# troyvvgroup/quemb

Hardware: AMD Instinct MI355X
Metric: fragment CCSD iters/sec (full BE sweep over synthetic n_occ=20 n_virt=200 fragments); corr-E error vs oracle in parity_max_abs_err_Eh / parity_n220_abs_err_Eh (higher is better)
Workload: dtype f64

## Files before the change

### include/qemb_hip_ops.h

```cpp
#ifndef QEMB_HIP_OPS_H
#define QEMB_HIP_OPS_H
#include "qemb_hip.h"
#ifdef __cplusplus
extern "C" {
#endif

#define QEMB_TIMER_LADDER 0
#define QEMB_TIMER_RINGS 1
#define QEMB_TIMER_ITER 2
#define QEMB_TIMER_AO2MO 3
#define QEMB_TIMER_SCF 4
#define QEMB_TIMER_GEMM_ANY 5
#define QEMB_TIMER_SCHMIDT 6
#define QEMB_TIMER_DF 7
int qemb_timer_begin(int slot);
int qemb_timer_end(int slot);
int qemb_timer_read(int slot, double* total_ms, int64_t* count);
int qemb_timer_reset(int slot);
int qemb_alloc_stats(long long* n_driver_allocs, long long* n_driver_frees, double* ms_in_driver_calls, double* gb_allocated, int reset);
int qemb_gemm_flop_count(double* flops, int reset);
int qemb_tape_cache_counters(int64_t* reused, int64_t* recorded, int reset);
int qemb_ctx_timer_read(int ctx, int slot, double* total_ms, int64_t* count, int reset);
int qemb_timer_live_events(int slot);

// ... 35 lines not shown
int qemb_op_unpack_s4(int64_t n, const double* s4, double* s1);
int qemb_op_pack_s4(int64_t n, const double* s1, double* s4);
int qemb_op_unpack_s8_to_s4(int64_t n, const double* s8, double* s4);
int qemb_op_mirror_lower(int64_t n, double* A, int64_t lda);
int qemb_op_k_from_pairs(int64_t n, const double* H, const double* D, double* K);
int qemb_op_jk_from_packed(int64_t n, const double* S4, const double* D, const double* Dp, double* Jp, double* K);
int qemb_op_pack_pm_cols(int64_t rows, int64_t v, const double* in, double* Op, int64_t ldp, double* Om, int64_t ldm);
int qemb_op_scatter_pm_rows(int64_t o, int64_t ncols, const double* Xp, const double* Xm, double* out);
int qemb_op_pack_w_pm(int64_t o, const double* W, double* Ap, int64_t lda_p, double* Am, int64_t lda_m);
int qemb_op_ladder_scatter_pm2(int64_t o, int64_t v, const double* Rp, int64_t ldp, const double* Rm, int64_t ldm, const double* Hp, const double* Hm,
                               int assign, double* t2);
int qemb_op_lincomb2(int64_t n, double a, const double* x, double b, const double* y, double beta, double* out);
int qemb_op_small_k_update(int64_t batch, int64_t M, int64_t N, int64_t K, double alpha, const double* A, int64_t sA, const double* B, int64_t sB, double* C, int64_t sC);
int qemb_op_ccsd_ph_layouts(int64_t o, int64_t v, const double* t2, const double* t1, double* T, double* Tp, double* S, double* Ut, double* Tpt, double* Th);
int qemb_op_ccsd_y_traces(int64_t o, int64_t v, const double* ZC, const double* ZB, double* Y);
int qemb_op_copy4_two(const int64_t dim[4], const double* in, const int64_t si[4], double* out, const int64_t so[4], double alpha, double beta, const double* base,
                      double* out2, const double* in2, double c2a, double c2b);
int qemb_op_scatter_pm_rows_add(int64_t o, int64_t ncols, const double* Xp, const double* Xm, double* out, const double* add);
int qemb_op_ccsd_y_traces_add(int64_t o, int64_t v, const double* ZC, const double* ZB, double* Y, const double* add);
int qemb_op_pack_w_pm_sum(int64_t o, const double* Wt, const double* X, const double* At, double* Ap, int64_t lda_p, double* Am, int64_t lda_m);
int qemb_op_ccsd_t1_small(int64_t o, int64_t v, const double* t1, const double* Lvv, const double* Loo, const double* Fov, double* t1n);
int qemb_op_ccsd_t1_assemble(int64_t o, int64_t v, const double* t1, const double* Lvv, const double* Loo, const double* Fov, const double* S, const double* Lph1,
                             const double* PA, int SA, int64_t strideA, const double* PB, int SB, int64_t strideB, double* t1n);
int qemb_op_gemv_rows_two(int64_t rows1, int64_t cols1, const double* T1, int64_t ld1, const double* x1, double* y1, double a1, double b1,
                          int64_t rows2, int64_t cols2, const double* T2, int64_t ld2, const double* x2, double* y2, double a2, double b2);
int qemb_op_ccsd_y_traces_slabs(int64_t o, int64_t v, const double* ZC, const double* ZB, double* Y, const double* add, int S, int64_t stride, double scale);
int qemb_op_gemv_rows2(int64_t rows, int64_t cols, const double* T1, int64_t ld1, const double* x1, const double* T2, int64_t ld2, const double* x2, double* y, double alpha, double beta);
int qemb_op_ccsd_finish_t2_rings(int64_t o, int64_t v, double* t2n, const double* U, const double* OV, const double* RS, const double* M, const double* eo, const double* ev, double* t1n);
int qemb_op_diis_push(int64_t n, const double* trial, const double* prev, double* e, double* xcopy, int m, const double* const* ys, int self, double* row_dev, double* row_host);
int qemb_op_ccsd_extrapolate_energy(int64_t o, int64_t v, int nterms, const double* coef, const double* const* xs, double* amp, const double* L, double* tau, double* e_host);
// ... 82 lines not shown
```

### quemb_amd/_lib.py

```python

from __future__ import annotations

import ctypes as C
import os
from pathlib import Path

import numpy as np

_HERE = Path(__file__).resolve().parent
LIB_PATH = _HERE / "libqemb_hip.so"

c_dp = C.POINTER(C.c_double)
c_i64 = C.c_int64
c_vp = C.c_void_p


QEMB_ERR_ARG, QEMB_ERR_ALLOC, QEMB_ERR_DEVICE, QEMB_ERR_NOCONV, QEMB_ERR_NUMERIC, QEMB_ERR_UNSUPPORTED = -1, -2, -3, -4, -5, -6


class QembError(RuntimeError):

    def __init__(self, msg="", status=None):
        super().__init__(msg)
        self.status = status
# ... 77 lines not shown
    f("qemb_op_unpack_s4", I, L, P, P)
    f("qemb_op_pack_s4", I, L, P, P)
    f("qemb_op_unpack_s8_to_s4", I, L, P, P)
    f("qemb_op_unpack_tril_rows", I, L, L, P, P)
    f("qemb_op_pack_pair_rows", I, L, L, P, P)
    f("qemb_op_mirror_lower", I, L, P, L)
    f("qemb_op_k_from_pairs", I, L, P, P, P)
    f("qemb_op_jk_from_packed", I, L, P, P, P, P, P)
    f("qemb_op_pack_pm_cols", I, L, L, P, P, L, P, L)
    f("qemb_op_scatter_pm_rows", I, L, L, P, P, P)
    f("qemb_op_pack_w_pm", I, L, P, P, L, P, L)
    f("qemb_op_ladder_scatter_pm2", I, L, L, P, L, P, L, P, P, I, P)
    f("qemb_op_lincomb2", I, L, D, P, D, P, D, P)
    f("qemb_op_small_k_update", I, L, L, L, L, D, P, L, P, L, P, L)
    f("qemb_op_ccsd_ph_layouts", I, L, L, P, P, P, P, P, P, P, P)
    f("qemb_op_ccsd_y_traces", I, L, L, P, P, P)
    f("qemb_op_copy4_two", I, C.POINTER(L), P, C.POINTER(L), P, C.POINTER(L), D, D, P, P, P, D, D)
    f("qemb_op_scatter_pm_rows_add", I, L, L, P, P, P, P)
    f("qemb_op_ccsd_y_traces_add", I, L, L, P, P, P, P)
    f("qemb_op_pack_w_pm_sum", I, L, P, P, P, P, L, P, L)
    f("qemb_op_ccsd_t1_small", I, L, L, P, P, P, P, P)
    f("qemb_op_gemv_rows2", I, L, L, P, L, P, P, L, P, P, D, D)
    f("qemb_op_ccsd_t1_assemble", I, L, L, P, P, P, P, P, P, P, I, L, P, I, L, P)
    f("qemb_op_gemv_rows_two", I, L, L, P, L, P, P, D, D, L, L, P, L, P, P, D, D)
    f("qemb_op_ccsd_y_traces_slabs", I, L, L, P, P, P, P, I, L, D)
    f("qemb_op_ccsd_finish_t2_rings", I, L, L, P, P, P, P, P, P, P, P)
    f("qemb_op_diis_push", I, L, P, P, P, P, I, P, I, P, P)
    f("qemb_op_ccsd_extrapolate_energy", I, L, L, I, P, P, P, P, P, P)
    f("qemb_op_gather_rows", I, L, L, P, P, L, P)
    f("qemb_op_scale_rows", I, L, L, P, P)
# ... 250 lines not shown
```

### quemb_amd/csrc/api.cpp

```cpp
#include <cstring>
#include <cstdlib>
#include <vector>
#include <execinfo.h>
#include <signal.h>
#include <unistd.h>
#include "../../include/qemb_hip_ops.h"
#include "dev_ops.h"
#include "ccsd.h"
#include "fragment.h"
#include "ao2mo.h"
#include "kdf.h"
#include "int3c.h"
#include "int4c.h"
#include "cd_core.h"
#include "loc_core.h"
#include "sci_core.h"
#include <algorithm>
#include <cmath>
#include <mutex>
#include <set>

using namespace qemb;
namespace qemb {
int dev_mfma_f64_peak(int iters, int blocks_per_cu, double* tflops);
// ... 183 lines not shown
int qemb_op_pack_w_pm(int64_t o, const double* W, double* Ap, int64_t lda_p, double* Am, int64_t lda_m) { return dev_pack_w_pm(o, W, Ap, lda_p, Am, lda_m); }
int qemb_op_ladder_scatter_pm2(int64_t o, int64_t v, const double* Rp, int64_t ldp, const double* Rm, int64_t ldm, const double* Hp, const double* Hm,
                               int assign, double* t2) { return dev_ladder_scatter_pm2(o, v, Rp, ldp, Rm, ldm, Hp, Hm, assign, t2); }
int qemb_op_lincomb2(int64_t n, double a, const double* x, double b, const double* y, double beta, double* out) {
  const double c[2] = {a, b};
  const double* xs[2] = {x, y};
  return dev_lincomb(n, 2, c, xs, beta, out);
}
int qemb_op_mirror_lower(int64_t n, double* A, int64_t lda) { return dev_mirror_lower(n, A, lda); }
int qemb_op_small_k_update(int64_t batch, int64_t M, int64_t N, int64_t K, double alpha, const double* A, int64_t sA, const double* B, int64_t sB, double* C, int64_t sC) {
  return dev_small_k_update(batch, M, N, K, alpha, A, sA, B, sB, C, sC);
}
int qemb_op_ccsd_ph_layouts(int64_t o, int64_t v, const double* t2, const double* t1, double* T, double* Tp, double* S, double* Ut, double* Tpt, double* Th) {
  return dev_ccsd_ph_layouts(o, v, t2, t1, T, Tp, S, Ut, Tpt, Th);
}
int qemb_op_copy4_two(const int64_t dim[4], const double* in, const int64_t si[4], double* out, const int64_t so[4], double alpha, double beta, const double* base,
                      double* out2, const double* in2, double c2a, double c2b) {
  Copy4Desc c{};
  for (int k = 0; k < 4; ++k) { c.dim[k] = dim[k]; c.si[k] = si[k]; c.so[k] = so[k]; }
  c.in = in; c.out = out; c.alpha = alpha; c.beta = beta; c.base = base;
  c.out2 = out2; c.in2 = in2; c.c2a = c2a; c.c2b = c2b;
  return dev_copy4(c);
}
int qemb_op_scatter_pm_rows_add(int64_t o, int64_t ncols, const double* Xp, const double* Xm, double* out, const double* add) { return dev_scatter_pm_rows(o, ncols, Xp, Xm, out, add); }
int qemb_op_ccsd_y_traces_add(int64_t o, int64_t v, const double* ZC, const double* ZB, double* Y, const double* add) { return dev_ccsd_y_traces(o, v, ZC, ZB, Y, add); }
int qemb_op_pack_w_pm_sum(int64_t o, const double* Wt, const double* X, const double* At, double* Ap, int64_t lda_p, double* Am, int64_t lda_m) {
  return dev_pack_w_pm_sum(o, Wt, X, At, Ap, lda_p, Am, lda_m);
}
int qemb_op_ccsd_t1_small(int64_t o, int64_t v, const double* t1, const double* Lvv, const double* Loo, const double* Fov, double* t1n) { return dev_ccsd_t1_small(o, v, t1, Lvv, Loo, Fov, t1n); }
int qemb_op_ccsd_t1_assemble(int64_t o, int64_t v, const double* t1, const double* Lvv, const double* Loo, const double* Fov, const double* S, const double* Lph1,
// ... 1064 lines not shown
```

### quemb_amd/csrc/ccsd.cpp

```cpp
#include "ccsd.h"
#include "ao2mo.h"
#include <algorithm>
#include <chrono>
#include <cmath>
#include <cstdio>
#include <cstdlib>
#include <cstring>
#include <string>

namespace qemb {

int mo_slab_ld(int n) { return (n >= 64 && n <= 1024) ? (n + 15) / 16 * 16 : n; }
int64_t mo_transform_work(int n) { return (int64_t)n * mo_slab_ld(n) * ((int64_t)n * (n + 1) / 2); }

static int mo_three_quarter_blocks(int n, int o, int nf, const double* T, int64_t slab, MoIntegrals& out, bool build_T34) {
  const int v = n - o;
  if (nf > 0 && build_T34) {
    QTRY(out.T34.alloc((int64_t)n * n * n * nf));
    QTRY(dev_extract_pf_t(n, T, 0, 0, 0, 0, n, n, n, nf, out.T34, slab));
  } else if (nf > 0) {
    QTRY(out.A1.alloc((int64_t)v * o * v * nf));
    QTRY(out.A2.alloc((int64_t)o * o * v * nf));
    QTRY(dev_extract_pf_t(n, T, o, 0, o, 0, v, o, v, nf, out.A1, slab));
    QTRY(dev_extract_pf_t(n, T, 0, 0, o, 0, o, o, v, nf, out.A2, slab));
// ... 133 lines not shown
    QTRY(mo_blocks_from_pair_product(n, o, X1, X0, out));
    QTRY(lap_AO2MO.close());
    return 0;
  }
  QTRY(dev_unpack_tril_rows(np, n, X1, X0));
  if (nf > 0) {
    QTRY(gemm(np, (int64_t)nf * n, naux, 1.0, Lpk, np, false, Lh, n2, false, 0.0, X1, (int64_t)nf * n));
    QTRY(mo_three_quarter_blocks(n, o, nf, X1, (int64_t)nf * n, out, build_T34));
  }
  Lh.release(); Lpk.release();
  QTRY(mo_blocks_from_pair_first(n, o, X0, X1, mo_transform_work(n), out, build_Vl));
  QTRY(lap_AO2MO.close());
  return 0;
}

int CcsdSolver::setup(MoIntegrals&& ints, const double* mo_energy_dev) {
  I_ = std::move(ints);
  o_ = I_.o; v_ = I_.v; nf_ = I_.nf;
  const int64_t o = o_, v = v_, nov = o * v, oo = o * o, vv = v * v, N2 = oo * vv;
  QTRY(eo_.alloc(o)); QTRY(ev_.alloc(v));
  QTRY(dev_d2d(eo_, mo_energy_dev, sizeof(double) * o));
  QTRY(dev_d2d(ev_, mo_energy_dev + o, sizeof(double) * v));
  QTRY(ovov_t_.alloc(nov * nov)); QTRY(Lovov_.alloc(nov * nov)); QTRY(Loovv_.alloc(N2)); QTRY(OVoovv_.alloc(N2));
  QTRY(Lovoo_.alloc(o * v * oo)); QTRY(W1base_.alloc(N2)); QTRY(W2base_.alloc(N2)); QTRY(Lph1_.alloc(N2));
  QTRY(oooo_p_.alloc(oo * oo));
  QTRY(perm4(ovov_t_, I_.ovov, o, v, o, v, 0, 3, 2, 1));
  QTRY(dcopy(nov * nov, I_.ovov, Lovov_));
  QTRY(axpby(nov * nov, -1.0, ovov_t_, 2.0, Lovov_));
  QTRY(perm4(Loovv_, Lovov_, o, v, o, v, 0, 2, 1, 3));
  QTRY(perm4(OVoovv_, I_.ovov, o, v, o, v, 0, 2, 1, 3));
// ... 25 lines not shown
    if (I_.ovvv_pk.p) ovvv_pk_ = std::move(I_.ovvv_pk);
    else { QTRY(ovvv_pk_.alloc(o * v * npv)); QTRY(dev_pack_tril_rows(o * v, v, I_.ovvv, ovvv_pk_)); }
  }
  QTRY(Gp_.alloc(oo * I_.ldp)); QTRY(Gm_.alloc(oo * I_.ldm));
  QTRY(dev_pack_pm_cols(oo, v, OVoovv_, Gp_, I_.ldp, Gm_, I_.ldm));
  QTRY(perm4(oooo_p_, I_.oooo, o, o, o, o, 1, 3, 0, 2));
  QTRY(ovoo_cikl_.alloc(v * oo * o));
  QTRY(perm4(ovoo_cikl_, I_.ovoo, o, v, o, o, 1, 3, 2, 0));
  const int64_t na = nov + N2;
  QTRY(amp_.alloc(na)); QTRY(ampn_.alloc(na)); QTRY(diff_.alloc(na));
  for (DBuf* b : {&tau_, &T_, &Tp_, &S_, &W1_, &W2_, &W12_, &W12b_, &R_, &U_}) QTRY(b->alloc(N2));
  const int64_t NG = std::max<int64_t>(N2, oo * o * v);
  QTRY(G2_.alloc(NG));
  plans_ = ccsd_gemm_plans(o, v);
  QTRY(Fvv_.alloc(plans_.fvv.elems()));
  QTRY(T1P_.alloc(plans_.pa.elems() + plans_.pb.elems()));
  QTRY(Foo_.alloc(oo)); QTRY(Fov_.alloc(nov)); QTRY(Z_.alloc(oo)); QTRY(Y_.alloc(vv));
  QTRY(Ytmp_.alloc(vv)); QTRY(Loo_.alloc(oo)); QTRY(Lvv_.alloc(vv)); QTRY(Q_.alloc(oo)); QTRY(Wo_.alloc(oo * oo));
  QTRY(O1_.alloc(oo * oo)); QTRY(X_.alloc(oo * nov)); QTRY(scal_.alloc(8));
  {
    const int64_t npo = o * (o + 1) / 2, nmo = std::max<int64_t>(o * (o - 1) / 2, 1);
    QTRY(LTp_.alloc(npo * I_.ldp)); QTRY(LRp_.alloc(std::max(npo * I_.ldp, plans_.ladder_p.elems())));
    QTRY(LTm_.alloc(nmo * I_.ldm)); QTRY(LRm_.alloc(std::max(nmo * I_.ldm, plans_.ladder_m.elems())));
    QTRY(Xp_.alloc(plans_.x_p.elems())); QTRY(Xm_.alloc(plans_.x_m.elems()));
    QTRY(Xwp_.alloc(plans_.xw_p.elems())); QTRY(Xwm_.alloc(plans_.xw_m.elems())); QTRY(Xw_.alloc(oo * oo));
    lwp_ = npo + (npo & 1); lwm_ = std::max<int64_t>(2, nmo + (nmo & 1));
    QTRY(WAp_.alloc(npo * lwp_)); QTRY(WAm_.alloc(nmo * lwm_)); QTRY(HRp_.alloc(npo * I_.ldp)); QTRY(HRm_.alloc(nmo * I_.ldm));
    QTRY(ZB_.alloc(N2)); QTRY(ZC_.alloc(N2));
  }
  first_ = true;
  return 0;
// ... 70 lines not shown
}
static GemmPlan pick_xw_split(int64_t rows, int64_t oo, int64_t K) {
  if (K < 2048) return GemmPlan(rows, oo, K, -1, 0);
  const int cfg = GEMM_64x64;
  const int64_t tiles = gemm_tile_count(cfg, rows, oo);
  return GemmPlan(rows, oo, K, cfg, (int)std::max<int64_t>(1, std::min<int64_t>(std::min<int64_t>(64, K / 256), (512 + tiles - 1) / tiles)));
}
static GemmPlan pick_long_k(int64_t M, int64_t N, int64_t K, int cfg, bool many_slices = false) {
  if (cfg < 0) return GemmPlan(M, N, K, cfg, 0);
  int ks = gemm_auto_ksplit(gemm_tile_count(cfg, M, N), K);
  if (many_slices && ks > 1 && M <= 32 && N <= 32) ks = (int)std::min<int64_t>(512, K / 64);
  return GemmPlan(M, N, K, cfg, ks);
}
static int tile_tall(int64_t o) { return (o <= 32) ? GEMM_128x32 : -1; }
static int tile_wide(int64_t o) { return (o <= 32) ? GEMM_32x128 : -1; }

CcsdGemmPlans ccsd_gemm_plans(int64_t o, int64_t v) {
  int64_t ldp, ldm;
  packed_pair_lds(v, ldp, ldm);
  const int64_t oo = o * o, vv = v * v, nov = o * v;
  const int64_t npo = o * (o + 1) / 2, nmo = std::max<int64_t>(o * (o - 1) / 2, 1), npv = v * (v + 1) / 2, nmv = std::max<int64_t>(v * (v - 1) / 2, 1);
  CcsdGemmPlans p;
  p.fvv = pick_long_k(v, v, oo * v, (v <= 256) ? GEMM_64x64 : -1);
  p.pa = pick_long_k(o, v, o * vv, tile_wide(o), true);
  p.pb = pick_long_k(o, v, o * v * o, tile_wide(o), true);
  p.ladder_p = pick_pair_gemm(npo, npv, ldp);
  p.ladder_m = pick_pair_gemm(nmo, nmv, ldm);
  p.xw_p = pick_xw_split(npo, oo, ldp);
  p.xw_m = pick_xw_split(nmo, oo, ldm);
  p.x_p = pick_pair_gemm(npo, nov, ldp, true);
// ... 25 lines not shown
      if (nmo > 0 && nmv > 0) QTRY(gemm(nmo, nmv, nmo, 1.0, WAm_, lwm_, true, LTm_, ldm, false, 0.0, HRm_, ldm, 1, 0, 0, 0, nmv >= 2048 ? tile_for(nmo) : -1));
      QTRY(dev_region_end());
      QTRY(dev_ladder_scatter_pm2(o, v, LRp_, sp.ld, LRm_, sm.ld, HRp_, (nmo > 0 && nmv > 0) ? HRm_.p : nullptr, 1, out, sp.S, sp.stride, sm.S, sm.stride, ldp, ldm));
    } else {
      QTRY(dev_ladder_scatter_pm2(o, v, LRp_, sp.ld, LRm_, sm.ld, nullptr, nullptr, 0, out, sp.S, sp.stride, sm.S, sm.stride));
    }
  }
  return 0;
}

int CcsdSolver::update_amps(double* t1n, double* t2n) {
  const int64_t o = o_, v = v_, nov = o * v, oo = o * o, vv = v * v;
  const double* t1 = this->t1();
  const double* t2 = this->t2();
  QTRY(dev_region_begin());
  QTRY(dev_ccsd_ph_layouts(o, v, t2, t1, T_, Tp_, S_, W12_, W12b_, R_));
  QTRY(dev_region_chain());
  QTRY(dev_ladder_pack_tau(o, v, tau_, LTp_, I_.ldp, LTm_, I_.ldm));
  QTRY(dev_region_end());

  {
    const int64_t nmo = o * (o - 1) / 2, nmv = v * (v - 1) / 2;
    SlabGemm sp, sm;
    QTRY(dev_region_begin());
    QTRY(gemm_slabs(plans_.xw_p, LTp_, I_.ldp, Gp_, I_.ldp, Xwp_, oo, sp));
    QTRY(dev_region_chain());
    if (nmo > 0) {
      if (nmv > 0) QTRY(gemm_slabs(plans_.xw_m, LTm_, I_.ldm, Gm_, I_.ldm, Xwm_, oo, sm));
      else QTRY(dev_fill(Xwm_, nmo * oo, 0.0));
    }
    QTRY(dev_region_end());
    QTRY(dev_scatter_pm_rows(o, oo, Xwp_, Xwm_, Xw_, nullptr, sp.S, sp.stride, sm.S, sm.stride));
  }
  QTRY(dev_foo_from_x(o, Xw_, Loo_));
  SlabGemm sfvv;
  double fvv_scale = -1.0;
  if (plans_.fvv.ks > 1) QTRY(gemm_slabs(plans_.fvv, tau_, v, Loovv_, v, Fvv_, v, sfvv, false, false));
  else { QTRY(gemm(v, v, oo * v, -1.0, tau_, v, false, Loovv_, v, false, 0.0, Fvv_, v, 1, 0, 0, 0, plans_.fvv.cfg)); fvv_scale = 1.0; }
  QTRY(dev_gemv_rows_two(nov, nov, Lovov_, nov, t1, Fov_, 1.0, 0.0, oo, nov, LovooT_, nov, t1, Loo_, 1.0, 1.0));
  const int cfg_tall = tile_tall(o), cfg_wide = tile_wide(o);
  QTRY(dev_region_begin());
  QTRY(gemm(o * vv, o, v, 1.0, I_.ovvv, v, true, t1, v, true, 0.0, ZB_, o, 1, 0, 0, 0, cfg_tall));
  QTRY(dev_region_chain());
  {
    const int64_t npv = v * (v + 1) / 2;
    const bool vec_ok = (npv % 2) == 0;
    QTRY(gemm(o, npv, v, 1.0, t1, v, true, ovvv_pk_, npv, false, 0.0, ZCp_, npv, o, 0, v * npv, o * npv, vec_ok ? cfg_wide : -1));
    QTRY(dev_unpack_tril_rows(oo, v, ZCp_, ZC_));
  }
  QTRY(dev_region_end());
  QTRY(dev_ccsd_y_traces(o, v, ZC_, ZB_, Lvv_, Fvv_, sfvv.S, sfvv.stride, fvv_scale));

  SlabGemm spa, spb;
  double* PA = T1P_.p;
  QTRY(dev_region_begin());
  QTRY(gemm_slabs(plans_.pa, R_, o * vv, I_.ovvv, v, PA, v, spa, true, false));
  double* PB = PA + (int64_t)spa.S * nov;
  QTRY(dev_region_chain());
  QTRY(gemm_slabs(plans_.pb, Lovoo_, o, T_, v, PB, v, spb, false, false));
  QTRY(dev_region_end());
  QTRY(dev_ccsd_t1_assemble(o, v, t1, Lvv_, Loo_, Fov_, S_, Lph1_, PA, spa.S, nov, PB, spb.S, nov, t1n));

  QTRY(gemm(o, oo * o, v, 1.0, t1, v, true, ovoo_cikl_, oo * o, false, 0.0, O1_, oo * o));
  QTRY(dev_pack_w_pm_sum(o, oooo_p_, Xw_, O1_, WAp_, lwp_, WAm_, lwm_));
  QTRY(apply_ladder(tau_, t2n, true, true));

  QTRY(gemm(oo * v, v, v, 1.0, t2, v, true, Lvv_, v, true, 0.0, U_, v));
  QTRY(gemm(o, o * vv, o, -1.0, Loo_, o, false, t2, o * vv, false, 1.0, U_, o * vv, 1, 0, 0, 0, cfg_wide));
  {
    const int64_t nmo = o * (o - 1) / 2;
    SlabGemm sp, sm;
    QTRY(dev_region_begin());
    QTRY(gemm_slabs(plans_.x_p, LTp_, I_.ldp, OVp_, I_.ldp, Xp_, nov, sp));
    QTRY(dev_region_chain());
    if (nmo > 0) QTRY(gemm_slabs(plans_.x_m, LTm_, I_.ldm, OVm_, I_.ldm, Xm_, nov, sm));
// ... 324 lines not shown
```

### quemb_amd/csrc/ccsd.h

```cpp
#pragma once
#include <cstdint>
#include <vector>
#include "dev_ops.h"
#include "tensor_utils.h"

namespace qemb {

struct CcsdOptions {
  double conv_tol = 1e-10;
  double conv_tol_normt = 1e-8;
  int max_cycle = 100;
  int diis_space = 6;
  int verbose = 0;
};

struct MoIntegrals {
  int n = 0, o = 0, v = 0, nf = 0;
  DBuf oooo, ovoo, ovov, oovv, ovvo, ovvv;
  DBuf ovvv_pk;
  DBuf Vl;
  DBuf Vp, Vm;
  int64_t ldp = 0, ldm = 0;
  DBuf A1, A2;
  DBuf T34;
// ... 45 lines not shown
  int64_t n_amp() const { return (int64_t)o_ * v_ + (int64_t)o_ * o_ * v_ * v_; }

 private:
  int update_amps(double* t1n, double* t2n);
  bool replay_regime() const;
  int record_update(bool as_tape, bool* began);
  int energy(const double* t1, const double* t2, double* e);
  int make_tau(const double* t1, const double* t2, double* tau);

  int o_ = 0, v_ = 0, nf_ = 0;
  MoIntegrals I_;
  DBuf eo_, ev_;
  DBuf ovov_t_, Lovov_, Loovv_, OVoovv_, Lovoo_, ovoo_ijka_, ovoo_kilc_, W1base_, W2base_, Lph1_, OVp_, OVm_, oooo_p_, ovoo_cikl_;
  DBuf amp_, ampn_, diff_;
  DBuf tau_, T_, Tp_, S_, W1_, W2_, W12_, W12b_, R_, U_, G2_, T1P_;
  DBuf LTp_, LTm_, LRp_, LRm_;
  DBuf Xp_, Xm_;
  DBuf ovvv_pk_, ZCp_;
  DBuf Gp_, Gm_;
  DBuf Xwp_, Xwm_, Xw_;
  DBuf WAp_, WAm_, HRp_, HRm_;
  int64_t lwp_ = 0, lwm_ = 0;
  DBuf ZB_, ZC_;
  CcsdGemmPlans plans_;
  DBuf Foo_, Fvv_, Fov_, Z_, Y_, Ytmp_, Loo_, Lvv_, Q_, Wo_, O1_, X_, scal_, LovooT_;
  std::vector<DeviceDIIS> diis_;
  bool first_ = true;
  dev_graph_t graph_ = nullptr;
  dev_tape_t tape_ = nullptr;
  int eager_iters_ = 0;
// ... 25 lines not shown
```

### quemb_amd/csrc/dev_ops.h

```cpp
#pragma once
#include <cstddef>
#include <cstdint>
#include <string>
#include "../../include/qemb_hip_ops.h"
#include "gemm_tiles.h"
#include "env.h"

namespace qemb {

void set_error(const std::string& msg);
const char* last_error();

#define QTRY(expr)              \
  do {                          \
    int _rc = (expr);           \
    if (_rc != 0) return _rc;   \
  } while (0)


int dev_init(int device);
int dev_sync();
int dev_sync_device();
int dev_ctx_count(int n);
int dev_ctx_bind(int k);
// ... 159 lines not shown
int dev_ccsd_finish_t2(int64_t o, int64_t v, double* t2n, const double* U, const double* OV, const double* eo, const double* ev);
int dev_ccsd_finish_t2_rings(int64_t o, int64_t v, double* t2n, const double* U, const double* OV, const double* RS, const double* M, const double* eo, const double* ev, double* t1n);
int dev_ladder_scatter_pm(int64_t o, int64_t v, const double* Rp, int64_t ldp, const double* Rm, int64_t ldm, double* t2);
int dev_ladder_scatter_pm2(int64_t o, int64_t v, const double* Rp, int64_t ldp, const double* Rm, int64_t ldm, const double* Hp, const double* Hm,
                           int assign, double* t2, int Sp = 1, int64_t strideP = 0, int Sm = 1, int64_t strideM = 0, int64_t ldhp = 0, int64_t ldhm = 0);
int dev_pack_w_pm(int64_t o, const double* W, double* Ap, int64_t lda_p, double* Am, int64_t lda_m);
int dev_pack_w_pm_sum(int64_t o, const double* Wt, const double* X, const double* At, double* Ap, int64_t lda_p, double* Am, int64_t lda_m);
int dev_ccsd_t1_small(int64_t o, int64_t v, const double* t1, const double* Lvv, const double* Loo, const double* Fov, double* t1n);
int dev_ccsd_t1_assemble(int64_t o, int64_t v, const double* t1, const double* Lvv, const double* Loo, const double* Fov, const double* S, const double* Lph1,
                         const double* PA, int SA, int64_t strideA, const double* PB, int SB, int64_t strideB, double* t1n);
int dev_gemv_rows_two(int64_t rows1, int64_t cols1, const double* T1, int64_t ld1, const double* x1, double* y1, double a1, double b1,
                      int64_t rows2, int64_t cols2, const double* T2, int64_t ld2, const double* x2, double* y2, double a2, double b2);
int dev_gemv_rows2(int64_t rows, int64_t cols, const double* T1, int64_t ld1, const double* x1, const double* T2, int64_t ld2, const double* x2, double* y, double alpha, double beta);
int dev_foo_from_x(int64_t o, const double* X, double* F);
int dev_ccsd_ph_layouts(int64_t o, int64_t v, const double* t2, const double* t1, double* T, double* Tp, double* S, double* Ut, double* Tpt, double* Th);
int dev_small_k_update(int64_t batch, int64_t M, int64_t N, int64_t K, double alpha, const double* A, int64_t sA, const double* B, int64_t sB,
                       double* C, int64_t sC);
int dev_ccsd_y_traces(int64_t o, int64_t v, const double* ZC, const double* ZB, double* Y, const double* add = nullptr, int S = 1, int64_t stride = 0, double scale = 1.0);

inline int64_t dev_mp2_partial_count(int64_t o, int64_t v) {
  const int64_t nt = (v + 31) / 32, oo = o * o;
  return nt * (nt + 1) / 2 * (oo < 4096 ? oo : 4096);
}
int dev_mp2_amplitudes(int64_t o, int64_t v, const double* ovov, const double* eo, const double* ev, double* t2, double* G, double* partials, double* e_dev);

inline int rdm2_check_args(int kind, int64_t o, int64_t v, const double* t1, const double* t2, const double* out) {
  if (kind != QEMB_RDM2_CCSD && kind != QEMB_RDM2_MP2) { set_error("dev_rdm2_assemble: kind must be QEMB_RDM2_CCSD or QEMB_RDM2_MP2"); return QEMB_ERR_ARG; }
  if (o <= 0 || v < 0 || !out || (v > 0 && (!t2 || (kind == QEMB_RDM2_CCSD && !t1)))) { set_error("dev_rdm2_assemble: bad arguments"); return QEMB_ERR_ARG; }
  if (o + v > 32767) { set_error("dev_rdm2_assemble: n = " + std::to_string(o + v) + " is beyond any n^4 tensor"); return QEMB_ERR_ARG; }
  return 0;
// ... 143 lines not shown
```

### quemb_amd/csrc/dev_ops_hip.hip

```cpp
#include <hip/hip_runtime.h>
#include <chrono>
#include <atomic>
#include <algorithm>
#include <cstdint>
#include <cstdlib>
#include <cstring>
#include <map>
#include <thread>
#include <mutex>
#include <string>
#include <type_traits>
#include <vector>
#include "dev_ops.h"
#include "hip_common.h"
#include "grouped_launch.h"

namespace qemb {
static thread_local std::string g_err;
void set_error(const std::string& msg) { g_err = msg; }
const char* last_error() { return g_err.c_str(); }

struct TimerLap { hipEvent_t e0, e1; bool ended; };
struct TimerSlot { double total_ms = 0; int64_t count = 0; std::vector<TimerLap> pending; std::vector<std::pair<hipEvent_t, hipEvent_t>> spare; };
static constexpr size_t TIMER_MAX_PENDING = 64;
// ... 1070 lines not shown
  const long long b0 = tb * 32 - a;
#pragma unroll
  for (int r = 0; r < 4; ++r) {
    const long long b = b0 + ty + 8 * r, c = tc * 32 + tx;
    xt[ty + 8 * r][tx] = (b >= 0 && b < v && c < v) ? X[b * v + c] : 0.0;
  }
  __syncthreads();
#pragma unroll
  for (int r = 0; r < 4; ++r) {
    const long long c = tc * 32 + ty + 8 * r, b = b0 + tx;
    if (c < v && b >= 0 && b < v) {
      const double x = X[c * v + b];
      const double xp = xt[tx][ty + 8 * r];
      const double tt = 2.0 * t1[j * v + c] * t1[k * v + b];
      const long long off = ((k * v + c) * o + j) * v + b;
      T[off] = x;
      Tp[off] = xp;
      const double s = 2.0 * x - xp;
      S[off] = s;
      Ut[off] = s - tt;
      Tpt[off] = xp + tt;
      Th[((k * o + j) * v + c) * v + b] = 2.0 * xp - x;
    }
  }
}
__global__ void __launch_bounds__(256) ccsd_ph_layouts_kernel(long long o, long long v, const double* __restrict__ t2, const double* __restrict__ t1,
                                                              double* __restrict__ T, double* __restrict__ Tp, double* __restrict__ S,
                                                              double* __restrict__ Ut, double* __restrict__ Tpt, double* __restrict__ Th, int tiles) { ccsd_ph_layouts_kernel_body(block_id(), grid_dim(), o, v, t2, t1, T, Tp, S, Ut, Tpt, Th, tiles); }
static const Groupable<ccsd_ph_layouts_kernel_body, 256> reg_ccsd_ph_layouts(ccsd_ph_layouts_kernel);
int dev_ccsd_ph_layouts(int64_t o, int64_t v, const double* t2, const double* t1, double* T, double* Tp, double* S, double* Ut, double* Tpt, double* Th) {
  REQUIRE_INIT();
  if (o <= 0 || v <= 0) return QEMB_OK;
  if (o > 65535) { set_error("dev_ccsd_ph_layouts: too many occupied orbitals"); return QEMB_ERR_ARG; }
  const long long tiles_c = (v + 31) / 32, tiles = (v + 15 + 31) / 32;
  return launch("dev_ccsd_ph_layouts", ccsd_ph_layouts_kernel, dim3((unsigned)(tiles_c * tiles), (unsigned)o, (unsigned)o), dim3(256), 0, g_stream, o, v, t2, t1,
                T, Tp, S, Ut, Tpt, Th, (int)tiles);
}

__device__ __forceinline__ void small_k_update_kernel_body(const uint3 BID, const uint3 GDIM, long long M, long long N, long long K, double alpha, const double* __restrict__ A, long long sA,
                                                             const double* __restrict__ B, long long sB, double* __restrict__ C, long long sC, int tiles_n) {
  __shared__ double As[32][33], Bs[32][33];
  const int tx = threadIdx.x & 31, ty = threadIdx.x >> 5;
  const long long tm = BID.x / tiles_n, tn = BID.x % tiles_n;
  const long long m0 = tm * 32, n0 = tn * 32;
  {
    const long long z = BID.y;
    const double* __restrict__ Az = A + z * sA;
    const double* __restrict__ Bz = B + z * sB;
    double* __restrict__ Cz = C + z * sC;
    double acc[4] = {0.0, 0.0, 0.0, 0.0};
    for (long long k0 = 0; k0 < K; k0 += 32) {
// ... 1919 lines not shown
```

Baseline: 57.45.

## Fuse the two ovvv contractions into one persistent MFMA pass over ovvv

Adds a persistent f64 MFMA kernel that streams each ovvv slab once through double-buffered LDS. It computes both the t1 contraction (ZB) and the Th contraction (per-block partial PA slabs) in that one read, replacing two separate GEMMs that each read the large ovvv tensor. The particle-hole layout kernel gains a variant that skips writing T and Th, and the PB GEMM now reads t2 directly against a pre-permuted Lovoo copy. The path is limited to shapes with o≤32 and may be off in the replay regime. It adds an extra Lovoo buffer and a one-block-per-CU schedule whose load balance depends on the shape.

```diff
diff --git a/include/qemb_hip_ops.h b/include/qemb_hip_ops.h
--- a/include/qemb_hip_ops.h
+++ b/include/qemb_hip_ops.h
@@ -73,6 +73,9 @@
 int qemb_op_small_k_update(int64_t batch, int64_t M, int64_t N, int64_t K, double alpha, const double* A, int64_t sA, const double* B, int64_t sB, double* C, int64_t sC);
 int qemb_op_ccsd_ph_layouts(int64_t o, int64_t v, const double* t2, const double* t1, double* T, double* Tp, double* S, double* Ut, double* Tpt, double* Th);
 int qemb_op_ccsd_y_traces(int64_t o, int64_t v, const double* ZC, const double* ZB, double* Y);
+int qemb_op_ccsd_ph_layouts_ring(int64_t o, int64_t v, const double* t2, const double* t1, double* Tp, double* S, double* Ut, double* Tpt);
+int qemb_op_ccsd_ovvv_slabs(int64_t o, int64_t v);
+int qemb_op_ccsd_ovvv_pass(int64_t o, int64_t v, const double* ovvv, const double* t1, const double* Thk, double* ZB, double* PA);
 int qemb_op_copy4_two(const int64_t dim[4], const double* in, const int64_t si[4], double* out, const int64_t so[4], double alpha, double beta, const double* base,
                       double* out2, const double* in2, double c2a, double c2b);
 int qemb_op_scatter_pm_rows_add(int64_t o, int64_t ncols, const double* Xp, const double* Xm, double* out, const double* add);
diff --git a/quemb_amd/_lib.py b/quemb_amd/_lib.py
--- a/quemb_amd/_lib.py
+++ b/quemb_amd/_lib.py
@@ -115,6 +115,9 @@
     f("qemb_op_lincomb2", I, L, D, P, D, P, D, P)
     f("qemb_op_small_k_update", I, L, L, L, L, D, P, L, P, L, P, L)
     f("qemb_op_ccsd_ph_layouts", I, L, L, P, P, P, P, P, P, P, P)
+    f("qemb_op_ccsd_ph_layouts_ring", I, L, L, P, P, P, P, P, P)
+    f("qemb_op_ccsd_ovvv_slabs", I, L, L)
+    f("qemb_op_ccsd_ovvv_pass", I, L, L, P, P, P, P, P)
     f("qemb_op_ccsd_y_traces", I, L, L, P, P, P)
     f("qemb_op_copy4_two", I, C.POINTER(L), P, C.POINTER(L), P, C.POINTER(L), D, D, P, P, P, D, D)
     f("qemb_op_scatter_pm_rows_add", I, L, L, P, P, P, P)
diff --git a/quemb_amd/csrc/api.cpp b/quemb_amd/csrc/api.cpp
--- a/quemb_amd/csrc/api.cpp
+++ b/quemb_amd/csrc/api.cpp
@@ -221,6 +221,13 @@
 int qemb_op_ccsd_ph_layouts(int64_t o, int64_t v, const double* t2, const double* t1, double* T, double* Tp, double* S, double* Ut, double* Tpt, double* Th) {
   return dev_ccsd_ph_layouts(o, v, t2, t1, T, Tp, S, Ut, Tpt, Th);
 }
+int qemb_op_ccsd_ph_layouts_ring(int64_t o, int64_t v, const double* t2, const double* t1, double* Tp, double* S, double* Ut, double* Tpt) {
+  return dev_ccsd_ph_layouts_ring(o, v, t2, t1, Tp, S, Ut, Tpt);
+}
+int qemb_op_ccsd_ovvv_slabs(int64_t o, int64_t v) { return dev_ccsd_ovvv_slabs(o, v); }
+int qemb_op_ccsd_ovvv_pass(int64_t o, int64_t v, const double* ovvv, const double* t1, const double* Thk, double* ZB, double* PA) {
+  return dev_ccsd_ovvv_pass(o, v, ovvv, t1, Thk, ZB, PA);
+}
 int qemb_op_copy4_two(const int64_t dim[4], const double* in, const int64_t si[4], double* out, const int64_t so[4], double alpha, double beta, const double* base,
                       double* out2, const double* in2, double c2a, double c2b) {
   Copy4Desc c{};
diff --git a/quemb_amd/csrc/ccsd.cpp b/quemb_amd/csrc/ccsd.cpp
--- a/quemb_amd/csrc/ccsd.cpp
+++ b/quemb_amd/csrc/ccsd.cpp
@@ -171,6 +171,7 @@
   return 0;
 }
 
+static bool use_ovvv_pass(int64_t o, int64_t v, bool replay);
 int CcsdSolver::setup(MoIntegrals&& ints, const double* mo_energy_dev) {
   I_ = std::move(ints);
   o_ = I_.o; v_ = I_.v; nf_ = I_.nf;
@@ -226,7 +227,14 @@
   QTRY(G2_.alloc(NG));
   plans_ = ccsd_gemm_plans(o, v);
   QTRY(Fvv_.alloc(plans_.fvv.elems()));
-  QTRY(T1P_.alloc(plans_.pa.elems() + plans_.pb.elems()));
+  ovvv_pass_ = use_ovvv_pass(o, v, replay_regime());
+  ovvv_G_ = ovvv_pass_ ? dev_ccsd_ovvv_slabs(o, v) : 0;
+  if (ovvv_pass_ && ovvv_G_ <= 0) ovvv_pass_ = false;
+  if (ovvv_pass_) {
+    QTRY(LovooK_.alloc(o * v * oo));
+    QTRY(perm4(LovooK_, Lovoo_, o, v, o, o, 0, 2, 1, 3));
+  }
+  QTRY(T1P_.alloc((ovvv_pass_ ? (int64_t)ovvv_G_ * nov : plans_.pa.elems()) + plans_.pb.elems()));
   QTRY(Foo_.alloc(oo)); QTRY(Fov_.alloc(nov)); QTRY(Z_.alloc(oo)); QTRY(Y_.alloc(vv));
   QTRY(Ytmp_.alloc(vv)); QTRY(Loo_.alloc(oo)); QTRY(Lvv_.alloc(vv)); QTRY(Q_.alloc(oo)); QTRY(Wo_.alloc(oo * oo));
   QTRY(O1_.alloc(oo * oo)); QTRY(X_.alloc(oo * nov)); QTRY(scal_.alloc(8));
@@ -327,6 +335,11 @@
 }
 static int tile_tall(int64_t o) { return (o <= 32) ? GEMM_128x32 : -1; }
 static int tile_wide(int64_t o) { return (o <= 32) ? GEMM_32x128 : -1; }
+static bool use_ovvv_pass(int64_t o, int64_t v, bool replay) {
+  const long long sw = env_int("QEMB_OVVV_PASS", -1);
+  if (sw == 0 || !ccsd_ovvv_shape_ok(o, v)) return false;
+  return sw > 0 || !replay;
+}
 
 CcsdGemmPlans ccsd_gemm_plans(int64_t o, int64_t v) {
   int64_t ldp, ldm;
@@ -382,7 +395,8 @@
   const double* t1 = this->t1();
   const double* t2 = this->t2();
   QTRY(dev_region_begin());
-  QTRY(dev_ccsd_ph_layouts(o, v, t2, t1, T_, Tp_, S_, W12_, W12b_, R_));
+  if (ovvv_pass_) QTRY(dev_ccsd_ph_layouts_ring(o, v, t2, t1, Tp_, S_, W12_, W12b_));
+  else QTRY(dev_ccsd_ph_layouts(o, v, t2, t1, T_, Tp_, S_, W12_, W12b_, R_));
   QTRY(dev_region_chain());
   QTRY(dev_ladder_pack_tau(o, v, tau_, LTp_, I_.ldp, LTm_, I_.ldm));
   QTRY(dev_region_end());
@@ -407,8 +421,10 @@
   else { QTRY(gemm(v, v, oo * v, -1.0, tau_, v, false, Loovv_, v, false, 0.0, Fvv_, v, 1, 0, 0, 0, plans_.fvv.cfg)); fvv_scale = 1.0; }
   QTRY(dev_gemv_rows_two(nov, nov, Lovov_, nov, t1, Fov_, 1.0, 0.0, oo, nov, LovooT_, nov, t1, Loo_, 1.0, 1.0));
   const int cfg_tall = tile_tall(o), cfg_wide = tile_wide(o);
+  double* PA = T1P_.p;
   QTRY(dev_region_begin());
-  QTRY(gemm(o * vv, o, v, 1.0, I_.ovvv, v, true, t1, v, true, 0.0, ZB_, o, 1, 0, 0, 0, cfg_tall));
+  if (ovvv_pass_) QTRY(dev_ccsd_ovvv_pass(o, v, I_.ovvv, t1, S_, ZB_, PA));
+  else QTRY(gemm(o * vv, o, v, 1.0, I_.ovvv, v, true, t1, v, true, 0.0, ZB_, o, 1, 0, 0, 0, cfg_tall));
   QTRY(dev_region_chain());
   {
     const int64_t npv = v * (v + 1) / 2;
@@ -420,13 +436,19 @@
   QTRY(dev_ccsd_y_traces(o, v, ZC_, ZB_, Lvv_, Fvv_, sfvv.S, sfvv.stride, fvv_scale));
 
   SlabGemm spa, spb;
-  double* PA = T1P_.p;
-  QTRY(dev_region_begin());
-  QTRY(gemm_slabs(plans_.pa, R_, o * vv, I_.ovvv, v, PA, v, spa, true, false));
-  double* PB = PA + (int64_t)spa.S * nov;
-  QTRY(dev_region_chain());
-  QTRY(gemm_slabs(plans_.pb, Lovoo_, o, T_, v, PB, v, spb, false, false));
-  QTRY(dev_region_end());
+  double* PB = nullptr;
+  if (ovvv_pass_) {
+    spa.S = ovvv_G_; spa.stride = nov; spa.ld = v;
+    PB = PA + (int64_t)spa.S * nov;
+    QTRY(gemm_slabs(plans_.pb, LovooK_, o, t2, v, PB, v, spb, false, false));
+  } else {
+    QTRY(dev_region_begin());
+    QTRY(gemm_slabs(plans_.pa, R_, o * vv, I_.ovvv, v, PA, v, spa, true, false));
+    PB = PA + (int64_t)spa.S * nov;
+    QTRY(dev_region_chain());
+    QTRY(gemm_slabs(plans_.pb, Lovoo_, o, T_, v, PB, v, spb, false, false));
+    QTRY(dev_region_end());
+  }
   QTRY(dev_ccsd_t1_assemble(o, v, t1, Lvv_, Loo_, Fov_, S_, Lph1_, PA, spa.S, nov, PB, spb.S, nov, t1n));
 
   QTRY(gemm(o, oo * o, v, 1.0, t1, v, true, ovoo_cikl_, oo * o, false, 0.0, O1_, oo * o));
diff --git a/quemb_amd/csrc/ccsd.h b/quemb_amd/csrc/ccsd.h
--- a/quemb_amd/csrc/ccsd.h
+++ b/quemb_amd/csrc/ccsd.h
@@ -83,6 +83,9 @@
   DBuf ovov_t_, Lovov_, Loovv_, OVoovv_, Lovoo_, ovoo_ijka_, ovoo_kilc_, W1base_, W2base_, Lph1_, OVp_, OVm_, oooo_p_, ovoo_cikl_;
   DBuf amp_, ampn_, diff_;
   DBuf tau_, T_, Tp_, S_, W1_, W2_, W12_, W12b_, R_, U_, G2_, T1P_;
+  bool ovvv_pass_ = false;
+  int ovvv_G_ = 0;
+  DBuf LovooK_;
   DBuf LTp_, LTm_, LRp_, LRm_;
   DBuf Xp_, Xm_;
   DBuf ovvv_pk_, ZCp_;
diff --git a/quemb_amd/csrc/ccsd_ovvv_ops.hip b/quemb_amd/csrc/ccsd_ovvv_ops.hip
--- /dev/null
+++ b/quemb_amd/csrc/ccsd_ovvv_ops.hip
@@ -0,0 +1,229 @@
+#include <cstdint>
+#include "hip_common.h"
+
+namespace qemb {
+namespace ovvv_pass {
+
+typedef double d4 __attribute__((ext_vector_type(4)));
+typedef double d2 __attribute__((ext_vector_type(2)));
+
+constexpr int OV_BK = 32;
+constexpr int OV_LD = OV_BK + 2;
+constexpr int OV_T = 512;
+constexpr int OV_WAVES = OV_T / 64;
+constexpr int OV_MAXU = CCSD_OVVV_MAX_TILES / OV_WAVES;
+constexpr int OV_MAXCH = (16 * CCSD_OVVV_MAX_ROWT * (OV_BK / 2) + OV_T - 1) / OV_T;
+
+struct OvvvArgs {
+  const double* ovvv; const double* t1; const double* thk;
+  double* zb; double* pa;
+  int o, v, rt;
+  long long nslab;
+};
+
+template <int NT, bool VEC2>
+__global__ void __launch_bounds__(OV_T) ccsd_ovvv_pass_kernel(const OvvvArgs g) {
+  extern __shared__ __attribute__((aligned(16))) double ov_smem[];
+  const int o = g.o, v = g.v, RT = g.rt;
+  const int tid = threadIdx.x, lane = tid & 63, l15 = lane & 15, l4 = lane >> 4;
+  const int wave = __builtin_amdgcn_readfirstlane(tid >> 6);
+  const int rows = 16 * (RT + NT);
+  const int items = rows * (OV_BK / 2);
+  const int nch = (items + OV_T - 1) / OV_T;
+  double* const buf0 = ov_smem;
+  double* const buf1 = ov_smem + rows * OV_LD;
+
+  const long long G = gridDim.x, bid = blockIdx.x;
+  const long long s_beg = bid * g.nslab / G, s_end = (bid + 1) * g.nslab / G;
+  const int nchunk = (v + OV_BK - 1) / OV_BK;
+  const long long nstep = (s_end - s_beg) * nchunk;
+
+  const int units = RT * NT, per = (units + OV_WAVES - 1) / OV_WAVES;
+  const int u_beg = wave * per < units ? wave * per : units - 1;
+  const int cnt = (units - wave * per) < 0 ? 0 : ((units - wave * per) < per ? (units - wave * per) : per);
+  const int ct_beg = u_beg / RT, rt_beg = u_beg - ct_beg * RT;
+  auto next_tile = [&](int& rt, int& ct) { ++rt; if (rt == RT) { rt = 0; ct = ct + 1 < NT ? ct + 1 : ct; } };
+  int a_off[OV_MAXU], b_off[OV_MAXU];
+  {
+    int rt = rt_beg, ct = ct_beg;
+#pragma unroll
+    for (int j = 0; j < OV_MAXU; ++j) { a_off[j] = (16 * rt) * OV_LD; b_off[j] = (16 * (RT + ct)) * OV_LD; next_tile(rt, ct); }
+  }
+  d4 acc[OV_MAXU];
+#pragma unroll
+  for (int j = 0; j < OV_MAXU; ++j) acc[j] = d4{0.0, 0.0, 0.0, 0.0};
+
+  constexpr int PPR = OV_BK / 2;
+  const int p2 = (tid % PPR) * 2;
+  int row_off[OV_MAXCH], row_kind[OV_MAXCH];
+#pragma unroll
+  for (int c = 0; c < OV_MAXCH; ++c) {
+    int R = (tid + c * OV_T) / PPR;
+    R = R < rows ? R : rows - 1;
+    if (R < 16 * RT) { const int a = R < v ? R : v - 1; row_off[c] = a * v; row_kind[c] = 0; }
+    else {
+      int n = R - 16 * RT;
+      n = n < 2 * o ? n : 2 * o - 1;
+      row_kind[c] = n < o ? 1 : 2;
+      row_off[c] = (n < o ? n : n - o) * v;
+    }
+  }
+  double reg[OV_MAXCH][2];
+  int fetched_d = 0;
+  auto fetch = [&](long long s, int k0) {
+    const double* __restrict__ pA = g.ovvv + s * (long long)v * v;
+    const double* __restrict__ pT = g.thk + s * (long long)o * v;
+    const int d = k0 + p2;
+    fetched_d = d;
+#pragma unroll
+    for (int c = 0; c < OV_MAXCH; ++c) {
+      const double* __restrict__ src = (row_kind[c] == 0 ? pA : row_kind[c] == 1 ? g.t1 : pT) + row_off[c];
+      if constexpr (VEC2) {
+        const int dc = d < v ? d : v - 2;
+        const d2 x = *reinterpret_cast<const d2*>(src + dc);
+        reg[c][0] = x[0];
+        reg[c][1] = x[1];
+      } else {
+        const int d0 = d < v ? d : v - 1, d1 = d + 1 < v ? d + 1 : v - 1;
+        reg[c][0] = src[d0];
+        reg[c][1] = src[d1];
+      }
+    }
+  };
+  auto stash = [&](double* __restrict__ S) {
+    const bool in0 = fetched_d < v, in1 = fetched_d + 1 < v;
+#pragma unroll
+    for (int c = 0; c < OV_MAXCH; ++c) {
+      const int item = tid + c * OV_T;
+      if (c < nch && item < items) *reinterpret_cast<d2*>(S + (item / PPR) * OV_LD + p2) = d2{in0 ? reg[c][0] : 0.0, in1 ? reg[c][1] : 0.0};
+    }
+  };
+
+  if (nstep > 0) {
+    fetch(s_beg, 0);
+    stash(buf0);
+    __syncthreads();
+    long long s = s_beg;
+    int ch = 0;
+    for (long long t = 0; t < nstep; ++t) {
+      {
+        const bool last = (t + 1 == nstep);
+        const bool wrap = (ch + 1 == nchunk);
+        const long long sn = last ? s : (wrap ? s + 1 : s);
+        const int chn = last ? ch : (wrap ? 0 : ch + 1);
+        fetch(sn, chn * OV_BK);
+      }
+      const double* __restrict__ S = (t & 1) ? buf1 : buf0;
+      const int kleft = v - ch * OV_BK;
+      const int nks = ((kleft < OV_BK ? kleft : OV_BK) + 3) >> 2;
+      const double* __restrict__ frag = S + l15 * OV_LD + l4;
+      auto load_frags = [&](double (&bf)[OV_MAXU], double (&af)[OV_MAXU], int ks) {
+#pragma unroll
+        for (int j = 0; j < OV_MAXU; ++j) { af[j] = frag[a_off[j] + 4 * ks]; bf[j] = frag[b_off[j] + 4 * ks]; }
+      };
+      auto mfmas = [&](const double (&bf)[OV_MAXU], const double (&af)[OV_MAXU]) {
+#pragma unroll
+        for (int j = 0; j < OV_MAXU; ++j)
+          if (j < cnt) acc[j] = __builtin_amdgcn_mfma_f64_16x16x4f64(af[j], bf[j], acc[j], 0, 0, 0);
+      };
+      double bf0[OV_MAXU], af0[OV_MAXU], bf1[OV_MAXU], af1[OV_MAXU];
+      load_frags(bf0, af0, 0);
+      for (int ks = 0; ks < nks; ks += 2) {
+        load_frags(bf1, af1, ks + 1 < nks ? ks + 1 : nks - 1);
+        mfmas(bf0, af0);
+        if (ks + 1 < nks) {
+          load_frags(bf0, af0, ks + 2 < nks ? ks + 2 : nks - 1);
+          mfmas(bf1, af1);
+        }
+      }
+      if (ch + 1 == nchunk) {
+        double* __restrict__ zb = g.zb + s * (long long)v * o;
+        int rt = rt_beg, ct = ct_beg;
+#pragma unroll
+        for (int j = 0; j < OV_MAXU; ++j) {
+          if (j < cnt && 16 * ct < o) {
+            const int i = 16 * ct + l15;
+#pragma unroll
+            for (int r = 0; r < 4; ++r) {
+              const int a = 16 * rt + l4 + 4 * r;
+              if (a < v && i < o) zb[(long long)a * o + i] = acc[j][r];
+              acc[j][r] = (i < o) ? 0.0 : acc[j][r];
+            }
+          }
+          next_tile(rt, ct);
+        }
+        ch = 0; ++s;
+      } else {
+        ++ch;
+      }
+      stash((t & 1) ? buf0 : buf1);
+      __syncthreads();
+    }
+  }
+  double* __restrict__ pa = g.pa + bid * (long long)o * v;
+  int rt = rt_beg, ct = ct_beg;
+#pragma unroll
+  for (int j = 0; j < OV_MAXU; ++j) {
+    if (j < cnt) {
+      const int i = 16 * ct + l15 - o;
+#pragma unroll
+      for (int r = 0; r < 4; ++r) {
+        const int a = 16 * rt + l4 + 4 * r;
+        if (a < v && i >= 0 && i < o) pa[(long long)i * v + a] = acc[j][r];
+      }
+    }
+    next_tile(rt, ct);
+  }
+}
+
+size_t ovvv_lds_bytes(int64_t o, int64_t v) {
+  const int64_t rt = (v + 15) / 16, nt = (2 * o + 15) / 16;
+  return (size_t)(2 * 16 * (rt + nt) * OV_LD) * sizeof(double);
+}
+
+template <int NT, bool VEC2>
+int launch_ovvv(const OvvvArgs& a, int G, size_t lds, hipStream_t st) {
+  auto kern = ccsd_ovvv_pass_kernel<NT, VEC2>;
+  static bool attr_set = false;
+  if (!attr_set) {
+    HIP_TRY(hipFuncSetAttribute((const void*)kern, hipFuncAttributeMaxDynamicSharedMemorySize, (int)(CCSD_OVVV_MAX_ROWT * 2 * 16 * OV_LD * sizeof(double))));
+    attr_set = true;
+  }
+  return launch("dev_ccsd_ovvv_pass", kern, dim3((unsigned)G), dim3(OV_T), lds, st, a);
+}
+
+}
+using namespace ovvv_pass;
+
+int dev_ccsd_ovvv_slabs(int64_t o, int64_t v) {
+  if (!ccsd_ovvv_shape_ok(o, v)) return 0;
+  static const int ncu = [] {
+    int dev = 0, n = 0;
+    if (hipGetDevice(&dev) != hipSuccess || hipDeviceGetAttribute(&n, hipDeviceAttributeMultiprocessorCount, dev) != hipSuccess || n <= 0) { (void)hipGetLastError(); n = 256; }
+    return n;
+  }();
+  return ncu;
+}
+
+int dev_ccsd_ovvv_pass(int64_t o, int64_t v, const double* ovvv, const double* t1, const double* Thk, double* ZB, double* PA) {
+  hipStream_t st = hip_stream();
+  if (!st) { set_error("libqemb_hip: call qemb_init(device) first"); return QEMB_ERR_DEVICE; }
+  if (!ccsd_ovvv_shape_ok(o, v)) { set_error("dev_ccsd_ovvv_pass: shape outside the kernel's limits (ccsd_ovvv_shape_ok)"); return QEMB_ERR_ARG; }
+  if (!ovvv || !t1 || !Thk || !ZB || !PA) { set_error("dev_ccsd_ovvv_pass: bad arguments"); return QEMB_ERR_ARG; }
+  const int G = dev_ccsd_ovvv_slabs(o, v);
+  OvvvArgs a{ovvv, t1, Thk, ZB, PA, (int)o, (int)v, (int)((v + 15) / 16), (long long)(o * v)};
+  const size_t lds = ovvv_lds_bytes(o, v);
+  const int nt = (int)((2 * o + 15) / 16);
+  const bool vec2 = (v % 2) == 0 && (((uintptr_t)ovvv | (uintptr_t)t1 | (uintptr_t)Thk) & 15) == 0;
+#define QEMB_OVVV_CASE(N)                                                                                  \
+  if (nt == N) return vec2 ? launch_ovvv<N, true>(a, G, lds, st) : launch_ovvv<N, false>(a, G, lds, st);
+  QEMB_OVVV_CASE(1)
+  QEMB_OVVV_CASE(2)
+  QEMB_OVVV_CASE(3)
+  QEMB_OVVV_CASE(4)
+#undef QEMB_OVVV_CASE
+  set_error("dev_ccsd_ovvv_pass: no kernel for this n_occ");
+  return QEMB_ERR_ARG;
+}
+
+}
diff --git a/quemb_amd/csrc/ccsd_ovvv_ops_hostcheck.cpp b/quemb_amd/csrc/ccsd_ovvv_ops_hostcheck.cpp
--- /dev/null
+++ b/quemb_amd/csrc/ccsd_ovvv_ops_hostcheck.cpp
@@ -0,0 +1,43 @@
+#ifdef QEMB_HOSTCHECK
+#include <algorithm>
+#include "dev_ops.h"
+
+namespace qemb {
+
+int dev_ccsd_ovvv_slabs(int64_t o, int64_t v) { return ccsd_ovvv_shape_ok(o, v) ? 6 : 0; }
+
+int dev_ccsd_ovvv_pass(int64_t o, int64_t v, const double* ovvv, const double* t1, const double* Thk, double* ZB, double* PA) {
+  if (!ccsd_ovvv_shape_ok(o, v)) { set_error("dev_ccsd_ovvv_pass: shape outside the kernel's limits (ccsd_ovvv_shape_ok)"); return QEMB_ERR_ARG; }
+  if (!ovvv || !t1 || !Thk || !ZB || !PA) { set_error("dev_ccsd_ovvv_pass: bad arguments"); return QEMB_ERR_ARG; }
+  const int64_t G = dev_ccsd_ovvv_slabs(o, v), nslab = o * v;
+  for (int64_t g = 0; g < G; ++g) {
+    double* pa = PA + g * o * v;
+    std::fill(pa, pa + o * v, 0.0);
+    for (int64_t s = g * nslab / G; s < (g + 1) * nslab / G; ++s) {
+      const double* A = ovvv + s * v * v;
+      const double* Th = Thk + s * o * v;
+      for (int64_t a = 0; a < v; ++a) for (int64_t i = 0; i < o; ++i) {
+        double zb = 0.0, p = 0.0;
+        for (int64_t d = 0; d < v; ++d) { zb += A[a * v + d] * t1[i * v + d]; p += A[a * v + d] * Th[i * v + d]; }
+        ZB[(s * v + a) * o + i] = zb;
+        pa[i * v + a] += p;
+      }
+    }
+  }
+  return 0;
+}
+
+int dev_ccsd_ph_layouts_ring(int64_t o, int64_t v, const double* t2, const double* t1, double* Tp, double* S, double* Ut, double* Tpt) {
+  for (int64_t k = 0; k < o; ++k) for (int64_t j = 0; j < o; ++j) for (int64_t c = 0; c < v; ++c) for (int64_t b = 0; b < v; ++b) {
+    const double x = t2[((k * o + j) * v + c) * v + b], xp = t2[((k * o + j) * v + b) * v + c], tt = 2.0 * t1[j * v + c] * t1[k * v + b];
+    const int64_t off = ((k * v + c) * o + j) * v + b;
+    Tp[off] = xp;
+    S[off] = 2.0 * x - xp;
+    Ut[off] = 2.0 * x - xp - tt;
+    Tpt[off] = xp + tt;
+  }
+  return 0;
+}
+
+}
+#endif
diff --git a/quemb_amd/csrc/dev_ops.h b/quemb_amd/csrc/dev_ops.h
--- a/quemb_amd/csrc/dev_ops.h
+++ b/quemb_amd/csrc/dev_ops.h
@@ -197,6 +197,16 @@
 int dev_gemv_rows2(int64_t rows, int64_t cols, const double* T1, int64_t ld1, const double* x1, const double* T2, int64_t ld2, const double* x2, double* y, double alpha, double beta);
 int dev_foo_from_x(int64_t o, const double* X, double* F);
 int dev_ccsd_ph_layouts(int64_t o, int64_t v, const double* t2, const double* t1, double* T, double* Tp, double* S, double* Ut, double* Tpt, double* Th);
+int dev_ccsd_ph_layouts_ring(int64_t o, int64_t v, const double* t2, const double* t1, double* Tp, double* S, double* Ut, double* Tpt);
+constexpr int CCSD_OVVV_MAX_TILES = 48;
+constexpr int CCSD_OVVV_MAX_ROWT = 18;
+inline bool ccsd_ovvv_shape_ok(int64_t o, int64_t v) {
+  if (o < 1 || v < 1 || o > 32) return false;
+  const int64_t rt = (v + 15) / 16, nt = (2 * o + 15) / 16;
+  return rt * nt <= CCSD_OVVV_MAX_TILES && rt + nt <= CCSD_OVVV_MAX_ROWT;
+}
+int dev_ccsd_ovvv_slabs(int64_t o, int64_t v);
+int dev_ccsd_ovvv_pass(int64_t o, int64_t v, const double* ovvv, const double* t1, const double* Thk, double* ZB, double* PA);
 int dev_small_k_update(int64_t batch, int64_t M, int64_t N, int64_t K, double alpha, const double* A, int64_t sA, const double* B, int64_t sB,
                        double* C, int64_t sC);
 int dev_ccsd_y_traces(int64_t o, int64_t v, const double* ZC, const double* ZB, double* Y, const double* add = nullptr, int S = 1, int64_t stride = 0, double scale = 1.0);
diff --git a/quemb_amd/csrc/dev_ops_hip.hip b/quemb_amd/csrc/dev_ops_hip.hip
--- a/quemb_amd/csrc/dev_ops_hip.hip
+++ b/quemb_amd/csrc/dev_ops_hip.hip
@@ -1108,13 +1108,13 @@
       const double xp = xt[tx][ty + 8 * r];
       const double tt = 2.0 * t1[j * v + c] * t1[k * v + b];
       const long long off = ((k * v + c) * o + j) * v + b;
-      T[off] = x;
+      if (T) T[off] = x;
       Tp[off] = xp;
       const double s = 2.0 * x - xp;
       S[off] = s;
       Ut[off] = s - tt;
       Tpt[off] = xp + tt;
-      Th[((k * o + j) * v + c) * v + b] = 2.0 * xp - x;
+      if (Th) Th[((k * o + j) * v + c) * v + b] = 2.0 * xp - x;
     }
   }
 }
@@ -1122,13 +1122,20 @@
                                                               double* __restrict__ T, double* __restrict__ Tp, double* __restrict__ S,
                                                               double* __restrict__ Ut, double* __restrict__ Tpt, double* __restrict__ Th, int tiles) { ccsd_ph_layouts_kernel_body(block_id(), grid_dim(), o, v, t2, t1, T, Tp, S, Ut, Tpt, Th, tiles); }
 static const Groupable<ccsd_ph_layouts_kernel_body, 256> reg_ccsd_ph_layouts(ccsd_ph_layouts_kernel);
-int dev_ccsd_ph_layouts(int64_t o, int64_t v, const double* t2, const double* t1, double* T, double* Tp, double* S, double* Ut, double* Tpt, double* Th) {
+static int ccsd_ph_layouts_launch(int64_t o, int64_t v, const double* t2, const double* t1, double* T, double* Tp, double* S, double* Ut, double* Tpt, double* Th) {
   REQUIRE_INIT();
   if (o <= 0 || v <= 0) return QEMB_OK;
   if (o > 65535) { set_error("dev_ccsd_ph_layouts: too many occupied orbitals"); return QEMB_ERR_ARG; }
   const long long tiles_c = (v + 31) / 32, tiles = (v + 15 + 31) / 32;
   return launch("dev_ccsd_ph_layouts", ccsd_ph_layouts_kernel, dim3((unsigned)(tiles_c * tiles), (unsigned)o, (unsigned)o), dim3(256), 0, g_stream, o, v, t2, t1,
                 T, Tp, S, Ut, Tpt, Th, (int)tiles);
+}
+int dev_ccsd_ph_layouts(int64_t o, int64_t v, const double* t2, const double* t1, double* T, double* Tp, double* S, double* Ut, double* Tpt, double* Th) {
+  if (!T || !Th) { set_error("dev_ccsd_ph_layouts: null output"); return QEMB_ERR_ARG; }
+  return ccsd_ph_layouts_launch(o, v, t2, t1, T, Tp, S, Ut, Tpt, Th);
+}
+int dev_ccsd_ph_layouts_ring(int64_t o, int64_t v, const double* t2, const double* t1, double* Tp, double* S, double* Ut, double* Tpt) {
+  return ccsd_ph_layouts_launch(o, v, t2, t1, nullptr, Tp, S, Ut, Tpt, nullptr);
 }
 
 __device__ __forceinline__ void small_k_update_kernel_body(const uint3 BID, const uint3 GDIM, long long M, long long N, long long K, double alpha, const double* __restrict__ A, long long sA,
```

Result: faster. 58.09, median of 6 (+1.1%).
